# cloudflare/zkp-ecdsa

Measured on NVIDIA H100. Metric: ZKAttest proofs/sec, higher is better.
Workload: dtype u256/u258 (32-bit limbs, Montgomery)

## Files before the change

### zkp_ecdsa_b200/csrc/zk_curves.cuh

```cuda
#pragma once
#include "zk_field.cuh"

namespace zk {

#define WEI_PT P256Pt
#define WEI_AFF P256Aff
#define WEI_JAC P256Jac
#define WEI_F P256p
#define WEI_FN(n) p256_##n
#define WEI_B_MONT ZK_P256_B_MONT
#define WEI_GX_MONT ZK_P256_GX_MONT
#define WEI_GY_MONT ZK_P256_GY_MONT
#include "zk_weier.inc"
#undef WEI_PT
#undef WEI_AFF
#undef WEI_JAC
#undef WEI_F
#undef WEI_FN
#undef WEI_B_MONT
#undef WEI_GX_MONT
#undef WEI_GY_MONT

#if defined(ZKA_PG_WAR256)
#define WEI_PT WarPt
#define WEI_AFF WarAff
#define WEI_JAC WarJac
#define WEI_F Warp
#define WEI_FN(n) war_##n
#define WEI_B_MONT ZK_WAR_B_MONT
#define WEI_GX_MONT ZK_WAR_GX_MONT
#define WEI_GY_MONT ZK_WAR_GY_MONT
#include "zk_weier.inc"
#undef WEI_PT
#undef WEI_AFF
#undef WEI_JAC
#undef WEI_F
#undef WEI_FN
#undef WEI_B_MONT
#undef WEI_GX_MONT
#undef WEI_GY_MONT

enum : int { PGL = 8 };
using PGp = Warp;
using FpPG = FpWar;
using TomPt = WarPt;
using TomPre = WarAff;
using TompMsm = Warp;
using TompCommit = Warp;
ZK_HD void tom_set_identity(TomPt& p) { war_set_identity(p); }
ZK_HD void tom_from_affine(TomPt& p, const uint32_t* x, const uint32_t* y) {
  copy_n<8>(p.x, x);
  copy_n<8>(p.y, y);
  Warp::set_one(p.z);
}
ZK_HD void tom_set_generator(TomPt& p) {
  WarAff g;
  war_set_generator(g);
  war_from_affine(p, g);
}
ZK_HD bool tom_on_curve(const uint32_t* x, const uint32_t* y) { return war_on_curve(x, y); }
ZK_HD void tom_add(TomPt& r, const TomPt& p, const TomPt& q) { war_add(r, p, q); }
template <bool kNeedT, class F = Warp>
ZK_HD void tom_madd(TomPt& r, const TomPt& p, const TomPre& q) { war_madd(r, p, q); }
ZK_HD void tom_dbl(TomPt& r, const TomPt& p) { war_dbl(r, p); }
ZK_HD void tom_neg(TomPt& r, const TomPt& p) {
  copy_n<8>(r.x, p.x);
  Warp::neg(r.y, p.y);
  copy_n<8>(r.z, p.z);
}
ZK_HD void pg_dbl_n(TomPt& p, int c) { war_dbl_n(p, c); }
ZK_HD void pg_pre_neg(TomPre& q) { Warp::neg(q.y, q.y); }
ZK_HD bool pg_is_identity(const TomPt& p) { return war_is_identity(p); }
ZK_HD void pg_fixed_to_msm(TomPt&) {}
#else
struct TomPt {
  uint32_t x[9], y[9], t[9], z[9];
};
struct TomPre {
  uint32_t x[9], y[9], k[9];
};

ZK_HD void tom_const(uint32_t* r, int which) {
  constexpr uint32_t sa[9] = ZK_TOM_SQRTA_MONT;
  constexpr uint32_t isa[9] = ZK_TOM_INVSQRTA_MONT;
  constexpr uint32_t d1[9] = ZK_TOM_D1_MONT;
  constexpr uint32_t gx[9] = ZK_TOM_GX1_MONT;
  constexpr uint32_t gy[9] = ZK_TOM_GY_MONT;
  constexpr uint32_t s2[9] = ZK_TOM_SQRTND1_MONT;
  constexpr uint32_t is2[9] = ZK_TOM_INVSQRTND1_MONT;
  constexpr uint32_t dd2[9] = ZK_TOM_2D2_MONT;
  constexpr uint32_t isd[9] = ZK_TOM_INVSQRTND_MONT;
#pragma unroll
  for (int i = 0; i < 9; i++)
    r[i] = which == 0 ? sa[i] : which == 1 ? isa[i] : which == 2 ? d1[i] : which == 3 ? gx[i] : which == 4 ? gy[i]
           : which == 5 ? s2[i] : which == 6 ? is2[i] : which == 7 ? dd2[i] : isd[i];
}
enum { TOM_SQRTA = 0, TOM_INVSQRTA = 1, TOM_D1 = 2, TOM_GX1 = 3, TOM_GY = 4, TOM_SQRTND1 = 5, TOM_INVSQRTND1 = 6,
       TOM_2D2 = 7, TOM_INVSQRTND = 8 };

struct TompInl : Tomp {
  ZK_HD static void mul(uint32_t* r, const uint32_t* a, const uint32_t* b) {
#if defined(__CUDA_ARCH__) && !defined(ZKA_NO_PTX_MUL)
    ptx::tom_mul_body(r, a, b);
#else
    Tomp::mul(r, a, b);
#endif
  }
  ZK_HD static void sqr(uint32_t* r, const uint32_t* a) { mul(r, a, a); }
};
#if defined(ZKA_COMMIT_INLINE)
using TompCommit = TompInl;
#else
using TompCommit = Tomp;
#endif
#if defined(ZKA_MSM_INLINE)
using TompMsm = TompInl;
#else
using TompMsm = Tomp;
#endif

template <bool kNeedT, class F = Tomp>
ZK_HD void tom2_madd(TomPt& r, const TomPt& p, const TomPre& q) {
  uint32_t A[9], B[9], C[9], D[9], E[9], Fv[9], G[9], H[9];
  F::sub(A, p.y, p.x);
  F::mul(A, A, q.x);
  F::add(B, p.y, p.x);
  F::mul(B, B, q.y);
  F::mul(C, p.t, q.k);
  F::add(D, p.z, p.z);
  F::sub(E, B, A);
  F::sub(Fv, D, C);
  F::add(G, D, C);
  F::add(H, B, A);
  F::mul(r.x, E, Fv);
  F::mul(r.y, G, H);
  if (kNeedT) F::mul(r.t, E, H);
  F::mul(r.z, Fv, G);
}

ZK_HD void tom_set_identity(TomPt& p) {
  zero_n<9>(p.x);
  Tomp::set_one(p.y);
  zero_n<9>(p.t);
  Tomp::set_one(p.z);
}
ZK_HD void tom_from_affine(TomPt& p, const uint32_t* x1, const uint32_t* y) {
  copy_n<9>(p.x, x1);
  copy_n<9>(p.y, y);
  Tomp::mul(p.t, x1, y);
  Tomp::set_one(p.z);
}
ZK_HD void tom_set_generator(TomPt& p) {
  uint32_t gx[9], gy[9];
  tom_const(gx, TOM_GX1);
  tom_const(gy, TOM_GY);
  tom_from_affine(p, gx, gy);
}
ZK_HD bool tom_on_curve(const uint32_t* x1, const uint32_t* y) {
  using F = Tomp;
  uint32_t xx[9], yy[9], l[9], r[9], d1[9], one[9];
  F::sqr(xx, x1);
  F::sqr(yy, y);
  F::add(l, xx, yy);
  F::mul(r, xx, yy);
  tom_const(d1, TOM_D1);
  F::mul(r, r, d1);
  F::set_one(one);
  F::add(r, r, one);
  uint32_t d[9], o[9];
  F::sub(d, l, r);
  zero_n<9>(o);
  o[0] = 1;
  F::mul(d, d, o);
  uint32_t nz = 0, np = 0;
#pragma unroll
  for (int i = 0; i < 9; i++) { nz |= d[i]; np |= d[i] ^ FpTom::p(i); }
  return nz == 0 || np == 0;
}

ZK_HD void tom_add(TomPt& r, const TomPt& p, const TomPt& q) {
  using F = Tomp;
  uint32_t A[9], B[9], C[9], D[9], E[9], Fv[9], G[9], H[9], d1[9];
  tom_const(d1, TOM_D1);
  F::mul(A, p.x, q.x);
  F::mul(B, p.y, q.y);
  F::mul(C, p.t, q.t);
  F::mul(C, C, d1);
  F::mul(D, p.z, q.z);
  F::add(E, p.x, p.y);
  F::add(H, q.x, q.y);
  F::mul(E, E, H);
  F::sub(E, E, A);
  F::sub(E, E, B);
  F::sub(Fv, D, C);
  F::add(G, D, C);
  F::sub(H, B, A);
  F::mul(r.x, E, Fv);
  F::mul(r.y, G, H);
  F::mul(r.t, E, H);
  F::mul(r.z, Fv, G);
}
template <bool kNeedT, class F = Tomp>
ZK_HD void tom_madd(TomPt& r, const TomPt& p, const TomPre& q) {
  uint32_t A[9], B[9], C[9], E[9], Fv[9], G[9], H[9];
  F::mul(A, p.x, q.x);
  F::mul(B, p.y, q.y);
  F::mul(C, p.t, q.k);
  F::add(E, p.x, p.y);
  F::add(H, q.x, q.y);
  F::mul(E, E, H);
  F::sub(E, E, A);
  F::sub(E, E, B);
  F::sub(Fv, p.z, C);
  F::add(G, p.z, C);
  F::sub(H, B, A);
  F::mul(r.x, E, Fv);
  F::mul(r.y, G, H);
  if (kNeedT) F::mul(r.t, E, H);
  F::mul(r.z, Fv, G);
}
ZK_HD void tom_dbl(TomPt& r, const TomPt& p) {
  using F = Tomp;
  uint32_t A[9], B[9], C[9], E[9], G[9], Fv[9], H[9];
  F::sqr(A, p.x);
  F::sqr(B, p.y);
  F::sqr(C, p.z);
  F::add(C, C, C);
  F::add(E, p.x, p.y);
  F::sqr(E, E);
  F::sub(E, E, A);
  F::sub(E, E, B);
  F::add(G, A, B);
  F::sub(Fv, G, C);
  F::sub(H, A, B);
  F::mul(r.x, E, Fv);
  F::mul(r.y, G, H);
  F::mul(r.t, E, H);
  F::mul(r.z, Fv, G);
}
ZK_HD void tom_neg(TomPt& r, const TomPt& p) {
  Tomp::neg(r.x, p.x);
  copy_n<9>(r.y, p.y);
  Tomp::neg(r.t, p.t);
  copy_n<9>(r.z, p.z);
}


enum : int { PGL = 9 };
using PGp = Tomp;
using FpPG = FpTom;
ZK_HD void pg_dbl_n(TomPt& p, int c) {
  for (int i = 0; i < c; i++) tom_dbl(p, p);
}
ZK_HD void pg_pre_neg(TomPre& q) {
  Tomp::neg(q.x, q.x);
  Tomp::neg(q.k, q.k);
}
ZK_HD bool pg_is_identity(const TomPt& p) { return Tomp::is_zero(p.x) && Tomp::eq(p.y, p.z); }
ZK_HD void pg_fixed_to_msm(TomPt& f) {
  uint32_t cw[9], X[9], Y[9], Tt[9], Zp[9], c1[9];
  tom_const(c1, TOM_INVSQRTND1);
  Tomp::mul(cw, f.x, c1);
  Tomp::mul(X, cw, f.y);
  Tomp::sqr(Y, f.z);
  Tomp::mul(Tt, cw, f.z);
  Tomp::mul(Zp, f.z, f.y);
  copy_n<9>(f.x, X); copy_n<9>(f.y, Y); copy_n<9>(f.t, Tt); copy_n<9>(f.z, Zp);
}
#endif

}
```

### zkp_ecdsa_b200/csrc/zk_field_ptx.cuh

```cuda
#pragma once

#if defined(__CUDA_ARCH__)
namespace zk {
namespace ptx {

__device__ __forceinline__ void mac3(uint32_t& a0, uint32_t& a1, uint32_t& a2, uint32_t x, uint32_t y) {
  asm("mad.lo.cc.u32 %0, %3, %4, %0;\n\t"
      "madc.hi.cc.u32 %1, %3, %4, %1;\n\t"
      "addc.u32 %2, %2, 0;"
      : "+r"(a0), "+r"(a1), "+r"(a2)
      : "r"(x), "r"(y));
}
__device__ __forceinline__ void add3(uint32_t& a0, uint32_t& a1, uint32_t& a2, uint32_t lo, uint32_t hi) {
  asm("add.cc.u32 %0, %0, %3;\n\t"
      "addc.cc.u32 %1, %1, %4;\n\t"
      "addc.u32 %2, %2, 0;"
      : "+r"(a0), "+r"(a1), "+r"(a2)
      : "r"(lo), "r"(hi));
}
__device__ __forceinline__ void addw(uint32_t& a0, uint32_t& a1, uint32_t& a2, uint32_t w) {
  asm("add.cc.u32 %0, %0, %3;\n\t"
      "addc.cc.u32 %1, %1, 0;\n\t"
      "addc.u32 %2, %2, 0;"
      : "+r"(a0), "+r"(a1), "+r"(a2)
      : "r"(w));
}
__device__ __forceinline__ void subw(uint32_t& a0, uint32_t& a1, uint32_t& a2, uint32_t w) {
  asm("sub.cc.u32 %0, %0, %3;\n\t"
      "subc.cc.u32 %1, %1, 0;\n\t"
      "subc.u32 %2, %2, 0;"
      : "+r"(a0), "+r"(a1), "+r"(a2)
      : "r"(w));
}

__device__ __forceinline__ uint32_t shl_alu(uint32_t x, uint32_t n) {
  uint32_t r;
  asm("shf.l.clamp.b32 %0, %1, %2, %3;" : "=r"(r) : "r"(0u), "r"(x), "r"(n));
  return r;
}
__device__ __forceinline__ uint32_t shr_top_alu(uint32_t x, uint32_t n) {
  uint32_t r;
  asm("shf.l.clamp.b32 %0, %1, %2, %3;" : "=r"(r) : "r"(x), "r"(0u), "r"(n));
  return r;
}

__device__ __forceinline__ void tom_mul_body_ps(uint32_t* r, const uint32_t* a, const uint32_t* b) {
  constexpr int N = 9;
  constexpr uint32_t P0 = FpTom::p(0), P1 = FpTom::p(1), P2 = FpTom::p(2), P3 = FpTom::p(3), P7 = FpTom::p(7);
  static_assert(FpTom::p(4) == 2 && FpTom::p(5) == 0 && FpTom::p(6) == 4 && FpTom::p(8) == 3, "tom.p limb structure");
  uint32_t m[N], t[N];
  uint32_t a0 = 0, a1 = 0, a2 = 0;
#pragma unroll
  for (int k = 0; k < 2 * N; k++) {
#pragma unroll
    for (int i = 0; i < N; i++) {
      const int j = k - i;
      if (j >= 0 && j < N) mac3(a0, a1, a2, a[i], b[j]);
    }
#pragma unroll
    for (int i = 0; i < N; i++) {
      const int j = k - i;
      if (i < k && j >= 1 && j < N) {
        if (j == 1) mac3(a0, a1, a2, m[i], P1);
        else if (j == 2) mac3(a0, a1, a2, m[i], P2);
        else if (j == 3) mac3(a0, a1, a2, m[i], P3);
        else if (j == 7) mac3(a0, a1, a2, m[i], P7);
        else if (j == 4) add3(a0, a1, a2, shl_alu(m[i], 1), shr_top_alu(m[i], 1));
        else if (j == 6) add3(a0, a1, a2, shl_alu(m[i], 2), shr_top_alu(m[i], 2));
        else if (j == 8) { add3(a0, a1, a2, shl_alu(m[i], 1), shr_top_alu(m[i], 1)); add3(a0, a1, a2, m[i], 0u); }
      }
    }
    if (k < N) {
      m[k] = a0 * FpTom::kN0Inv;
      mac3(a0, a1, a2, m[k], P0);
    } else {
      t[k - N] = a0;
    }
    a0 = a1; a1 = a2; a2 = 0;
  }
#pragma unroll
  for (int i = 0; i < N; i++) r[i] = t[i];
}

template <int I, bool kFirst>
__device__ __forceinline__ void tom_row(uint32_t* A, uint32_t* Bq, uint32_t x, const uint32_t* b) {
  if (kFirst) {
    asm("mad.lo.cc.u32 %0, %9, %10, %0;\n\t"
        "madc.hi.cc.u32 %1, %9, %10, %1;\n\t"
        "madc.lo.cc.u32 %2, %9, %11, %2;\n\t"
        "madc.hi.cc.u32 %3, %9, %11, %3;\n\t"
        "madc.lo.cc.u32 %4, %9, %12, %4;\n\t"
        "madc.hi.cc.u32 %5, %9, %12, %5;\n\t"
        "madc.lo.cc.u32 %6, %9, %13, %6;\n\t"
        "madc.hi.cc.u32 %7, %9, %13, %7;\n\t"
        "addc.u32 %8, %8, 0;"
        : "+r"(Bq[I + 1]), "+r"(Bq[I + 2]), "+r"(Bq[I + 3]), "+r"(Bq[I + 4]), "+r"(Bq[I + 5]), "+r"(Bq[I + 6]),
          "+r"(Bq[I + 7]), "+r"(Bq[I + 8]), "+r"(Bq[I + 9])
        : "r"(x), "r"(b[1]), "r"(b[3]), "r"(b[5]), "r"(b[7]));
  } else {
    asm("add.cc.u32 %0, %0, %10;\n\t"
        "madc.lo.cc.u32 %1, %11, %12, %1;\n\t"
        "madc.hi.cc.u32 %2, %11, %12, %2;\n\t"
        "madc.lo.cc.u32 %3, %11, %13, %3;\n\t"
        "madc.hi.cc.u32 %4, %11, %13, %4;\n\t"
        "madc.lo.cc.u32 %5, %11, %14, %5;\n\t"
        "madc.hi.cc.u32 %6, %11, %14, %6;\n\t"
        "madc.lo.cc.u32 %7, %11, %15, %7;\n\t"
        "madc.hi.cc.u32 %8, %11, %15, %8;\n\t"
        "addc.u32 %9, %9, 0;"
        : "+r"(A[I]), "+r"(Bq[I + 1]), "+r"(Bq[I + 2]), "+r"(Bq[I + 3]), "+r"(Bq[I + 4]), "+r"(Bq[I + 5]),
          "+r"(Bq[I + 6]), "+r"(Bq[I + 7]), "+r"(Bq[I + 8]), "+r"(Bq[I + 9])
        : "r"(Bq[I]), "r"(x), "r"(b[1]), "r"(b[3]), "r"(b[5]), "r"(b[7]));
  }
  asm("mad.lo.cc.u32 %0, %11, %12, %0;\n\t"
      "madc.hi.cc.u32 %1, %11, %12, %1;\n\t"
      "madc.lo.cc.u32 %2, %11, %13, %2;\n\t"
      "madc.hi.cc.u32 %3, %11, %13, %3;\n\t"
      "madc.lo.cc.u32 %4, %11, %14, %4;\n\t"
      "madc.hi.cc.u32 %5, %11, %14, %5;\n\t"
      "madc.lo.cc.u32 %6, %11, %15, %6;\n\t"
      "madc.hi.cc.u32 %7, %11, %15, %7;\n\t"
      "madc.lo.cc.u32 %8, %11, %16, %8;\n\t"
      "madc.hi.u32 %9, %11, %16, %9;"
      : "+r"(A[I]), "+r"(A[I + 1]), "+r"(A[I + 2]), "+r"(A[I + 3]), "+r"(A[I + 4]), "+r"(A[I + 5]), "+r"(A[I + 6]),
        "+r"(A[I + 7]), "+r"(A[I + 8]), "+r"(A[I + 9]), "+r"(A[I + 10])
      : "r"(x), "r"(b[0]), "r"(b[2]), "r"(b[4]), "r"(b[6]), "r"(b[8]));
  const uint32_t m = A[I] * FpTom::kN0Inv;
  const uint32_t s1 = shl_alu(m, 1), t1 = shr_top_alu(m, 1), s2 = shl_alu(m, 2), t2 = shr_top_alu(m, 2);
  uint32_t lo3, hi3, lo7, hi7;
  asm("add.cc.u32 %0, %2, %3;\n\taddc.u32 %1, %4, 0;" : "=r"(lo3), "=r"(hi3) : "r"(s1), "r"(m), "r"(t1));
  asm("sub.cc.u32 %0, 0, %2;\n\tsubc.u32 %1, %3, %4;" : "=r"(lo7), "=r"(hi7) : "r"(s2), "r"(m), "r"(t2));
  constexpr uint32_t P0 = FpTom::p(0), P1 = FpTom::p(1), P2 = FpTom::p(2), P3 = FpTom::p(3);
  asm("mad.lo.cc.u32 %0, %11, %12, %0;\n\t"
      "madc.hi.cc.u32 %1, %11, %12, %1;\n\t"
      "madc.lo.cc.u32 %2, %11, %13, %2;\n\t"
      "madc.hi.cc.u32 %3, %11, %13, %3;\n\t"
      "addc.cc.u32 %4, %4, %14;\n\t"
      "addc.cc.u32 %5, %5, %15;\n\t"
      "addc.cc.u32 %6, %6, %16;\n\t"
      "addc.cc.u32 %7, %7, %17;\n\t"
      "addc.cc.u32 %8, %8, %18;\n\t"
      "addc.u32 %9, %9, %19;"
      : "+r"(A[I]), "+r"(A[I + 1]), "+r"(A[I + 2]), "+r"(A[I + 3]), "+r"(A[I + 4]), "+r"(A[I + 5]), "+r"(A[I + 6]),
        "+r"(A[I + 7]), "+r"(A[I + 8]), "+r"(A[I + 9]), "+r"(A[I + 10])
      : "r"(m), "r"(P0), "r"(P2), "r"(s1), "r"(t1), "r"(s2), "r"(t2), "r"(lo3), "r"(hi3));
  asm("mad.lo.cc.u32 %0, %9, %10, %0;\n\t"
      "madc.hi.cc.u32 %1, %9, %10, %1;\n\t"
      "madc.lo.cc.u32 %2, %9, %11, %2;\n\t"
      "madc.hi.cc.u32 %3, %9, %11, %3;\n\t"
      "addc.cc.u32 %4, %4, 0;\n\t"
      "addc.cc.u32 %5, %5, 0;\n\t"
      "addc.cc.u32 %6, %6, %12;\n\t"
      "addc.cc.u32 %7, %7, %13;\n\t"
      "addc.u32 %8, %8, 0;"
      : "+r"(Bq[I + 1]), "+r"(Bq[I + 2]), "+r"(Bq[I + 3]), "+r"(Bq[I + 4]), "+r"(Bq[I + 5]), "+r"(Bq[I + 6]),
        "+r"(Bq[I + 7]), "+r"(Bq[I + 8]), "+r"(Bq[I + 9])
      : "r"(m), "r"(P1), "r"(P3), "r"(lo7), "r"(hi7));
}
__device__ __forceinline__ void tom_mul_body(uint32_t* r, const uint32_t* a, const uint32_t* b) {
  static_assert(FpTom::p(4) == 2 && FpTom::p(5) == 0 && FpTom::p(6) == 4 && FpTom::p(7) == 0xfffffffcu && FpTom::p(8) == 3,
                "tom.p limb structure");
  uint32_t E[20], O[20];
#pragma unroll
  for (int i = 0; i < 20; i++) { E[i] = 0; O[i] = 0; }
  tom_row<0, true>(E, O, a[0], b);
  tom_row<1, false>(O, E, a[1], b);
  tom_row<2, false>(E, O, a[2], b);
  tom_row<3, false>(O, E, a[3], b);
  tom_row<4, false>(E, O, a[4], b);
  tom_row<5, false>(O, E, a[5], b);
  tom_row<6, false>(E, O, a[6], b);
  tom_row<7, false>(O, E, a[7], b);
  tom_row<8, false>(E, O, a[8], b);
  asm("add.cc.u32 %0, %9, %18;\n\t"
      "addc.cc.u32 %1, %10, %19;\n\t"
      "addc.cc.u32 %2, %11, %20;\n\t"
      "addc.cc.u32 %3, %12, %21;\n\t"
      "addc.cc.u32 %4, %13, %22;\n\t"
      "addc.cc.u32 %5, %14, %23;\n\t"
      "addc.cc.u32 %6, %15, %24;\n\t"
      "addc.cc.u32 %7, %16, %25;\n\t"
      "addc.u32 %8, %17, %26;"
      : "=r"(r[0]), "=r"(r[1]), "=r"(r[2]), "=r"(r[3]), "=r"(r[4]), "=r"(r[5]), "=r"(r[6]), "=r"(r[7]), "=r"(r[8])
      : "r"(E[9]), "r"(E[10]), "r"(E[11]), "r"(E[12]), "r"(E[13]), "r"(E[14]), "r"(E[15]), "r"(E[16]), "r"(E[17]),
        "r"(O[9]), "r"(O[10]), "r"(O[11]), "r"(O[12]), "r"(O[13]), "r"(O[14]), "r"(O[15]), "r"(O[16]), "r"(O[17]));
}

__device__ __forceinline__ void p256_mul_body(uint32_t* r, const uint32_t* a, const uint32_t* b) {
  constexpr int N = 8;
  uint32_t m[N], t[N + 1];
  uint32_t a0 = 0, a1 = 0, a2 = 0;
#pragma unroll
  for (int k = 0; k < 2 * N; k++) {
#pragma unroll
    for (int i = 0; i < N; i++) {
      const int j = k - i;
      if (j >= 0 && j < N) mac3(a0, a1, a2, a[i], b[j]);
    }
    if (k - 3 >= 0 && k - 3 < N) addw(a0, a1, a2, m[k - 3 < 0 ? 0 : (k - 3 >= N ? 0 : k - 3)]);
    if (k - 6 >= 0 && k - 6 < N) addw(a0, a1, a2, m[k - 6 < 0 ? 0 : (k - 6 >= N ? 0 : k - 6)]);
    if (k - 7 >= 0 && k - 7 < N) subw(a0, a1, a2, m[k - 7 < 0 ? 0 : (k - 7 >= N ? 0 : k - 7)]);
    if (k - 8 >= 0 && k - 8 < N) addw(a0, a1, a2, m[k - 8 < 0 ? 0 : (k - 8 >= N ? 0 : k - 8)]);
    if (k < N) {
      m[k] = a0;
      a0 = 0;
    } else {
      t[k - N] = a0;
    }
    a0 = a1; a1 = a2; a2 = (uint32_t)((int32_t)a2 >> 31);
  }
  t[N] = a0;
  uint32_t u[N];
  uint32_t br = sub_p<FpP256>(u, t);
  const bool ge = (t[N] != 0) || (br == 0);
#pragma unroll
  for (int i = 0; i < N; i++) r[i] = ge ? u[i] : t[i];
}

__device__ __forceinline__ void p256_sqr_body(uint32_t* r, const uint32_t* a) {
  constexpr int N = 8;
  uint32_t m[N], t[N + 1];
  uint32_t a0 = 0, a1 = 0, a2 = 0;
#pragma unroll
  for (int k = 0; k < 2 * N; k++) {
    if (k >= 1 && k <= 2 * N - 3) {
      uint32_t c0 = 0, c1 = 0, c2 = 0;
#pragma unroll
      for (int i = 0; i < N; i++) {
        const int j = k - i;
        if (i < j && j < N) mac3(c0, c1, c2, a[i], a[j]);
      }
      asm("add.cc.u32 %0, %0, %0;\n\t"
          "addc.cc.u32 %1, %1, %1;\n\t"
          "addc.u32 %2, %2, %2;\n\t"
          "add.cc.u32 %3, %3, %0;\n\t"
          "addc.cc.u32 %4, %4, %1;\n\t"
          "addc.u32 %5, %5, %2;"
          : "+r"(c0), "+r"(c1), "+r"(c2), "+r"(a0), "+r"(a1), "+r"(a2));
    }
    if ((k & 1) == 0 && k / 2 < N) mac3(a0, a1, a2, a[k / 2], a[k / 2]);
    if (k - 3 >= 0 && k - 3 < N) addw(a0, a1, a2, m[k - 3 < 0 ? 0 : (k - 3 >= N ? 0 : k - 3)]);
    if (k - 6 >= 0 && k - 6 < N) addw(a0, a1, a2, m[k - 6 < 0 ? 0 : (k - 6 >= N ? 0 : k - 6)]);
    if (k - 7 >= 0 && k - 7 < N) subw(a0, a1, a2, m[k - 7 < 0 ? 0 : (k - 7 >= N ? 0 : k - 7)]);
    if (k - 8 >= 0 && k - 8 < N) addw(a0, a1, a2, m[k - 8 < 0 ? 0 : (k - 8 >= N ? 0 : k - 8)]);
    if (k < N) {
      m[k] = a0;
      a0 = 0;
    } else {
      t[k - N] = a0;
    }
    a0 = a1; a1 = a2; a2 = (uint32_t)((int32_t)a2 >> 31);
  }
  t[N] = a0;
  uint32_t u[N];
  uint32_t br = sub_p<FpP256>(u, t);
  const bool ge = (t[N] != 0) || (br == 0);
#pragma unroll
  for (int i = 0; i < N; i++) r[i] = ge ? u[i] : t[i];
}

template <int I, bool kFirst>
__device__ __forceinline__ void p256_row(uint32_t* A, uint32_t* Bq, uint32_t x, const uint32_t* b) {
  if (kFirst) {
    asm("mad.lo.cc.u32 %0, %9, %10, %0;\n\t"
        "madc.hi.cc.u32 %1, %9, %10, %1;\n\t"
        "madc.lo.cc.u32 %2, %9, %11, %2;\n\t"
        "madc.hi.cc.u32 %3, %9, %11, %3;\n\t"
        "madc.lo.cc.u32 %4, %9, %12, %4;\n\t"
        "madc.hi.cc.u32 %5, %9, %12, %5;\n\t"
        "madc.lo.cc.u32 %6, %9, %13, %6;\n\t"
        "madc.hi.cc.u32 %7, %9, %13, %7;\n\t"
        "addc.u32 %8, %8, 0;"
        : "+r"(Bq[I + 1]), "+r"(Bq[I + 2]), "+r"(Bq[I + 3]), "+r"(Bq[I + 4]), "+r"(Bq[I + 5]), "+r"(Bq[I + 6]),
          "+r"(Bq[I + 7]), "+r"(Bq[I + 8]), "+r"(Bq[I + 9])
        : "r"(x), "r"(b[1]), "r"(b[3]), "r"(b[5]), "r"(b[7]));
  } else {
    asm("add.cc.u32 %0, %0, %10;\n\t"
        "madc.lo.cc.u32 %1, %11, %12, %1;\n\t"
        "madc.hi.cc.u32 %2, %11, %12, %2;\n\t"
        "madc.lo.cc.u32 %3, %11, %13, %3;\n\t"
        "madc.hi.cc.u32 %4, %11, %13, %4;\n\t"
        "madc.lo.cc.u32 %5, %11, %14, %5;\n\t"
        "madc.hi.cc.u32 %6, %11, %14, %6;\n\t"
        "madc.lo.cc.u32 %7, %11, %15, %7;\n\t"
        "madc.hi.cc.u32 %8, %11, %15, %8;\n\t"
        "addc.u32 %9, %9, 0;"
        : "+r"(A[I]), "+r"(Bq[I + 1]), "+r"(Bq[I + 2]), "+r"(Bq[I + 3]), "+r"(Bq[I + 4]), "+r"(Bq[I + 5]),
          "+r"(Bq[I + 6]), "+r"(Bq[I + 7]), "+r"(Bq[I + 8]), "+r"(Bq[I + 9])
        : "r"(Bq[I]), "r"(x), "r"(b[1]), "r"(b[3]), "r"(b[5]), "r"(b[7]));
  }
  asm("mad.lo.cc.u32 %0, %9, %10, %0;\n\t"
      "madc.hi.cc.u32 %1, %9, %10, %1;\n\t"
      "madc.lo.cc.u32 %2, %9, %11, %2;\n\t"
      "madc.hi.cc.u32 %3, %9, %11, %3;\n\t"
      "madc.lo.cc.u32 %4, %9, %12, %4;\n\t"
      "madc.hi.cc.u32 %5, %9, %12, %5;\n\t"
      "madc.lo.cc.u32 %6, %9, %13, %6;\n\t"
      "madc.hi.cc.u32 %7, %9, %13, %7;\n\t"
      "addc.u32 %8, %8, 0;"
      : "+r"(A[I]), "+r"(A[I + 1]), "+r"(A[I + 2]), "+r"(A[I + 3]), "+r"(A[I + 4]), "+r"(A[I + 5]), "+r"(A[I + 6]),
        "+r"(A[I + 7]), "+r"(A[I + 8])
      : "r"(x), "r"(b[0]), "r"(b[2]), "r"(b[4]), "r"(b[6]));
  const uint32_t m = A[I];
  uint32_t negm, third;
  asm("sub.cc.u32 %0, 0, %2;\n\tsubc.u32 %1, %2, 0;" : "=r"(negm), "=r"(third) : "r"(m));
  asm("add.cc.u32 %0, %0, %7;\n\t"
      "addc.cc.u32 %1, %1, 0;\n\t"
      "addc.cc.u32 %2, %2, 0;\n\t"
      "addc.cc.u32 %3, %3, %7;\n\t"
      "addc.cc.u32 %4, %4, %8;\n\t"
      "addc.cc.u32 %5, %5, %9;\n\t"
      "addc.u32 %6, %6, 0;"
      : "+r"(A[I + 3]), "+r"(A[I + 4]), "+r"(A[I + 5]), "+r"(A[I + 6]), "+r"(A[I + 7]), "+r"(A[I + 8]), "+r"(A[I + 9])
      : "r"(m), "r"(negm), "r"(third));
}
__device__ __forceinline__ void p256_mul_body_os(uint32_t* r, const uint32_t* a, const uint32_t* b) {
  constexpr int N = 8;
  uint32_t E[18], O[18];
#pragma unroll
  for (int i = 0; i < 18; i++) { E[i] = 0; O[i] = 0; }
  p256_row<0, true>(E, O, a[0], b);
  p256_row<1, false>(O, E, a[1], b);
  p256_row<2, false>(E, O, a[2], b);
  p256_row<3, false>(O, E, a[3], b);
  p256_row<4, false>(E, O, a[4], b);
  p256_row<5, false>(O, E, a[5], b);
  p256_row<6, false>(E, O, a[6], b);
  p256_row<7, false>(O, E, a[7], b);
  uint32_t t[N + 1];
  asm("add.cc.u32 %0, %9, %18;\n\t"
      "addc.cc.u32 %1, %10, %19;\n\t"
      "addc.cc.u32 %2, %11, %20;\n\t"
      "addc.cc.u32 %3, %12, %21;\n\t"
      "addc.cc.u32 %4, %13, %22;\n\t"
      "addc.cc.u32 %5, %14, %23;\n\t"
      "addc.cc.u32 %6, %15, %24;\n\t"
      "addc.cc.u32 %7, %16, %25;\n\t"
      "addc.u32 %8, %17, %26;"
// ... 68 lines not shown
```

### zkp_ecdsa_b200/csrc/zk_ops.cuh

```cuda
#pragma once
#include "zk_curves.cuh"
#include "zk_layout.h"
#include "zk_sha256.cuh"

namespace zk {

#if defined(__CUDA_ARCH__)
#define ZK_SET_STATUS(ptr, code) atomicCAS((int*)(ptr), 0, (int)(code))
#define ZK_SET_STATUS_OVER(ptr, code, over) \
  do {                                      \
    atomicCAS((int*)(ptr), 0, (int)(code)); \
    atomicCAS((int*)(ptr), (int)(over), (int)(code)); \
  } while (0)
#else
#define ZK_SET_STATUS_OVER(ptr, code, over)              \
  do {                                                   \
    if (*(ptr) == 0 || *(ptr) == (over)) *(ptr) = (code); \
  } while (0)
#define ZK_SET_STATUS(ptr, code) \
  do {                           \
    if (*(ptr) == 0) *(ptr) = (code); \
  } while (0)
#endif

// ... 342 lines not shown
      tom_add(acc, acc, p);
    }
  }
};
struct TomTabE2Task {
  const uint32_t* proj;
  uint32_t* pre;
  int count;
  ZK_HD void operator()(int t) const {
    using F = Tomp;
    constexpr int CH = 16;
    const int lo = t * CH;
    int n = count - lo;
    if (n > CH) n = CH;
    if (n <= 0) return;
    uint32_t pf[CH][9];
    uint32_t acc[9], y[9], z[9], den[9];
    F::set_one(acc);
    for (int k = 0; k < n; k++) {
      const uint32_t* src = proj + (size_t)(lo + k) * TOM_PROJ_WORDS;
      uint32_t xx[9];
      tom_ld_xyz(xx, y, z, src);
      F::mul(den, y, z);
      F::mul(acc, acc, den);
      copy_n<9>(pf[k], acc);
    }
    uint32_t inv[9], s2[9], dd2[9];
    F::inv(inv, acc);
    tom_const(s2, TOM_SQRTND1);
    tom_const(dd2, TOM_2D2);
    for (int k = n - 1; k >= 0; k--) {
      const uint32_t* src = proj + (size_t)(lo + k) * TOM_PROJ_WORDS;
      uint32_t x[9], di[9], w[9], v[9], kk[9], ym[9], yp[9];
      tom_ld_xyz(x, y, z, src);
      F::mul(den, y, z);
      if (k > 0) F::mul(di, inv, pf[k - 1]); else copy_n<9>(di, inv);
      F::mul(inv, inv, den);
      F::mul(w, x, y);
      F::mul(w, w, di);
      F::mul(w, w, s2);
      F::sqr(v, z);
      F::mul(v, v, di);
      F::mul(kk, w, v);
      F::mul(kk, kk, dd2);
      F::sub(ym, v, w);
      F::add(yp, v, w);
      F::reduce(ym); F::reduce(yp); F::reduce(kk);
      uint32_t* o = pre + (size_t)(lo + k) * TOM_PRE_WORDS;
      st<9>(o, ym); st<9>(o + 9, yp); st<9>(o + 18, kk);
      for (int i = 27; i < 32; i++) o[i] = 0;
    }
  }
};

struct TomNormTask {
  const uint32_t* proj;
  uint32_t* aff;
  uint8_t* bytes;
  int count;
  int chunk;
  int e2;
  int aff_mod, aff_lim;
  ZK_HD static void canon2p(uint32_t* r) {
    uint32_t t[9], p2[9];
#pragma unroll
    for (int i = 0; i < 9; i++) p2[i] = (FpTom::p(i) << 1) | (i > 0 ? (FpTom::p(i - 1) >> 31) : 0u);
    uint32_t br = sub_n<9>(t, r, p2);
    csel_n<9>(r, br == 0, t, r);
    br = sub_p<FpTom>(t, r);
    csel_n<9>(r, br == 0, t, r);
  }
  ZK_HD void operator()(int t) const {
    using F = Tomp;
    const int lo = t * chunk;
    int n = count - lo;
    if (n > chunk) n = chunk;
    if (n <= 0) return;
    uint32_t pre[NORM_CHUNK_MAX][9];
    uint32_t acc[9], z[9], v[9], den[9];
    F::set_one(acc);
    for (int k = 0; k < n; k++) {
      const uint32_t* src = proj + (size_t)(lo + k) * TOM_PROJ_WORDS;
      uint32_t xx[9];
      tom_ld_xyz(xx, v, z, src);
      if (e2) F::mul(den, z, v); else copy_n<9>(den, z);
      F::mul(acc, acc, den);
      copy_n<9>(pre[k], acc);
    }
    uint32_t inv[9], isa[9], is2[9], isd[9], one_plain[9];
    F::inv(inv, acc);
    tom_const(isa, TOM_INVSQRTA);
    tom_const(is2, TOM_INVSQRTND1);
    tom_const(isd, TOM_INVSQRTND);
    zero_n<9>(one_plain);
    one_plain[0] = 1;
    for (int k = n - 1; k >= 0; k--) {
      const uint32_t* src = proj + (size_t)(lo + k) * TOM_PROJ_WORDS;
      uint32_t X[9], Y[9], di[9];
      tom_ld_xyz(X, Y, z, src);
      if (e2) F::mul(den, z, Y); else copy_n<9>(den, z);
      if (k > 0) F::mul(di, inv, pre[k - 1]); else copy_n<9>(di, inv);
      F::mul(inv, inv, den);
      if (bytes) {
        uint32_t Dp[9], cx[9], cy[9];
        F::mul(Dp, di, one_plain);
        if (e2) {
          F::mul(cx, X, Y);
          F::mul(cx, cx, isd);
          F::mul(cx, cx, Dp);
          F::sqr(cy, z);
          F::mul(cy, cy, Dp);
        } else {
          F::mul(cx, X, isa);
          F::mul(cx, cx, Dp);
          F::mul(cy, Y, Dp);
        }
        canon2p(cx);
        canon2p(cy);
        store_point_words<9, 33>(bytes + (size_t)(lo + k) * BSTRIDE, 0x04u, cx, cy);
      }
      if (aff && ((lo + k) % aff_mod) < aff_lim) {
        uint32_t x[9], y[9];
        if (e2) {
          uint32_t zi[9], vi[9];
          F::mul(zi, di, Y);
          F::mul(vi, di, z);
          F::mul(x, X, zi);
          F::mul(x, x, is2);
          F::mul(y, z, vi);
        } else {
          F::mul(x, X, di);
          F::mul(y, Y, di);
        }
        uint32_t* a = aff + (size_t)(lo + k) * TOM_AFF_WORDS;
        st<9>(a, x);
        st<9>(a + 9, y);
      }
    }
  }
};

struct TomCommitTask {
  const uint32_t* jv;
  const uint32_t* jr;
  const uint32_t* gtab;
  const uint32_t* htab;
  uint32_t* proj;
  int w, nwin;
  ZK_HD void operator()(int t) const {
    uint32_t v[8], r[8];
    ld<8>(v, jv + (size_t)t * 8);
    ld<8>(r, jr + (size_t)t * 8);
    TomPt acc;
    tom_set_identity(acc);
    const size_t ne = (size_t)fb_entries(w);
    uint32_t cv = 0, cr = 0;
    for (int j = 0; j < nwin; j++) {
      TomPre q;
      bool nv, nr;
      const uint32_t dv = signed_digit(v, j, w, cv, nv), dr = signed_digit(r, j, w, cr, nr);
      tom_ld_pre(q, gtab + ((size_t)j * ne + dv) * TOM_PRE_WORDS);
      tom2_pre_neg(q, nv);
      tom2_madd<true>(acc, acc, q);
      tom_ld_pre(q, htab + ((size_t)j * ne + dr) * TOM_PRE_WORDS);
      tom2_pre_neg(q, nr);
      tom2_madd<true>(acc, acc, q);
    }
    uint32_t* o = proj + (size_t)t * TOM_PROJ_WORDS;
    tom_st_xyz(o, acc.x, acc.y, acc.z);
  }
};

struct TomCommitGTask {
  const uint32_t* jv;
  const uint32_t* gtab;
  uint32_t* ext;
  int w, nwin;
  ZK_HD void operator()(int t) const {
    const int item = t / GJOBS_PER_ITEM, g = t % GJOBS_PER_ITEM;
    uint32_t v[8];
    ld<8>(v, jv + ((size_t)item * JOBS_PER_ITEM + item_job_of_gpart(g)) * 8);
    TomPt acc;
    tom_set_identity(acc);
    const size_t ne = (size_t)fb_entries(w);
    uint32_t carry = 0;
#pragma unroll 1
    for (int j = 0; j < nwin; j++) {
      TomPre q;
      bool neg;
      const uint32_t d = signed_digit(v, j, w, carry, neg);
      tom_ld_pre(q, gtab + ((size_t)j * ne + d) * TOM_PRE_WORDS);
      tom2_pre_neg(q, neg);
      tom2_madd<true, TompCommit>(acc, acc, q);
    }
    uint32_t* o = ext + (size_t)t * TOM_EXT_WORDS;
    st<9>(o, acc.x); st<9>(o + 9, acc.y); st<9>(o + 18, acc.t); st<9>(o + 27, acc.z);
  }
};
struct TomCommitHTask {
  const uint32_t* jr;
  const uint32_t* htab;
  const uint32_t* ext;
  uint32_t* proj;
  int w, nwin;
  ZK_HD void operator()(int t) const {
    const int item = t / JOBS_PER_ITEM, jb = t % JOBS_PER_ITEM;
    uint32_t r[8];
    ld<8>(r, jr + (size_t)t * 8);
    TomPt acc;
    const uint32_t* s = ext + ((size_t)item * GJOBS_PER_ITEM + item_gpart_of_job(jb)) * TOM_EXT_WORDS;
    ld<9>(acc.x, s); ld<9>(acc.y, s + 9); ld<9>(acc.t, s + 18); ld<9>(acc.z, s + 27);
    const size_t ne = (size_t)fb_entries(w);
    uint32_t carry = 0;
#pragma unroll 1
    for (int j = 0; j < nwin; j++) {
      TomPre q;
      bool neg;
      const uint32_t d = signed_digit(r, j, w, carry, neg);
      tom_ld_pre(q, htab + ((size_t)j * ne + d) * TOM_PRE_WORDS);
      tom2_pre_neg(q, neg);
      tom2_madd<true, TompCommit>(acc, acc, q);
    }
    tom_st_xyz(proj + (size_t)t * TOM_PROJ_WORDS, acc.x, acc.y, acc.z);
  }
};

#if !defined(ZKA_HOSTSIM) && defined(ZKA_COMMIT_MINBLOCKS)
template <> struct TaskMinBlocks<TomCommitHTask> { static constexpr int value = ZKA_COMMIT_MINBLOCKS; };
template <> struct TaskMinBlocks<TomCommitGTask> { static constexpr int value = ZKA_COMMIT_MINBLOCKS; };
template <> struct TaskMinBlocks<TomCommitTask> { static constexpr int value = ZKA_COMMIT_MINBLOCKS; };
#endif

#endif

enum : int { GK_BLOCK_BITS = 10 };
ZK_HD int gk_block_bits(int n) { return n < GK_BLOCK_BITS ? n : GK_BLOCK_BITS; }
ZK_HD void gk_block_sum(uint32_t* acc, const uint32_t* ring_m, const uint32_t (*fz)[8], const uint32_t (*fo)[8], int n,
                        int k, uint32_t blk, const uint32_t* vw) {
  using F = Tomq;
  uint32_t P[21][8];
  F::set_one(P[n]);
  for (int j = n - 1; j >= k; j--) F::mul(P[j], P[j + 1], ((blk >> (j - k)) & 1u) ? fo[j] : fz[j]);
  for (int j = k - 1; j >= 0; j--) F::mul(P[j], P[j + 1], fz[j]);
  zero_n<8>(acc);
  const size_t base = (size_t)blk << k;
  const uint32_t cnt = 1u << k;
  for (uint32_t l = 0;;) {
    uint32_t vi[8], term[8];
    ld<8>(vi, ring_m + (base + l) * 8);
    if (vw) F::sub(vi, vw, vi);
    F::mul(term, vi, P[0]);
    F::add(acc, acc, term);
    l++;
    if (l == cnt) break;
    int tz = 0;
    while (!((l >> tz) & 1u)) tz++;
    F::mul(P[tz], P[tz + 1], fo[tz]);
    for (int j = tz - 1; j >= 0; j--) F::mul(P[j], P[j + 1], fz[j]);
  }
}

ZK_HD bool hash_pt_fetch(uint32_t* t, const uint8_t* p, int len) {
  if (((size_t)p & 3) || len < 64 || len > 68) return false;
  if (aligned16(p)) {
#pragma unroll
    for (int j = 0; j < 4; j++) ld4(t + 4 * j, p + 16 * j);
    t[16] = len > 64 ? *reinterpret_cast<const uint32_t*>(p + 64) : 0u;
    return true;
  }
  const uint32_t* q = reinterpret_cast<const uint32_t*>(p);
#pragma unroll
  for (int j = 0; j < 17; j++) t[j] = (4 * j < len) ? q[j] : 0u;
  return true;
}
template <class Src>
ZK_HD void hash_points80(uint32_t* c3, const Src& src, int npts) {
  Sha256 h;
  h.init();
  uint32_t nx[17], cu[17];
  int nlen = 0;
  const uint8_t* np = npts > 0 ? src(0, nlen) : nullptr;
  bool nfast = npts > 0 && hash_pt_fetch(nx, np, nlen);
  for (int i = 0; i < npts; i++) {
    const uint8_t* p = np;
    const int len = nlen;
    const bool fast = nfast;
#pragma unroll
    for (int j = 0; j < 17; j++) cu[j] = nx[j];
    if (i + 1 < npts) {
      np = src(i + 1, nlen);
      nfast = hash_pt_fetch(nx, np, nlen);
    }
    if (fast) h.feed17(cu, len);
    else h.update(p, len);
  }
  h.final80(c3);
}

ZK_HD void challenge_to_limbs(uint32_t* r, const uint32_t* c3) {
  zero_n<8>(r);
  r[0] = c3[0]; r[1] = c3[1]; r[2] = c3[2];
}

template <int N>
ZK_HD void load_point(uint32_t* w, const uint8_t* src) {
  if (aligned16(src)) {
#pragma unroll
    for (int j = 0; j < BSTRIDE / 16; j++) ld4(w + 4 * j, src + 16 * j);
  } else if (((size_t)src & 3) == 0) {
    const uint32_t* sw = reinterpret_cast<const uint32_t*>(src);
#pragma unroll
    for (int j = 0; j < BSTRIDE / 4; j++) w[j] = 4 * j < N ? sw[j] : 0u;
  } else {
#pragma unroll
    for (int j = 0; j < BSTRIDE / 4; j++) {
      uint32_t v = 0;
#pragma unroll
      for (int t = 0; t < 4; t++)
        if (4 * j + t < N) v |= (uint32_t)src[4 * j + t] << (8 * t);
      w[j] = v;
    }
  }
}

struct ByteWriter {
  uint8_t* blk;
  uint32_t q[4];
  int fill;
  int lead;
  ZK_HD explicit ByteWriter(uint8_t* dst) : blk(dst - ((size_t)dst & 15)), fill((int)((size_t)dst & 15)), lead(fill) {
    q[0] = q[1] = q[2] = q[3] = 0;
  }
  ZK_HD static uint32_t funnel(uint32_t lo, uint32_t hi, int sh) {
#if defined(__CUDA_ARCH__)
    return __funnelshift_l(lo, hi, sh);
#else
    return (uint32_t)((((uint64_t)hi << 32) | lo) >> (32 - sh));
#endif
  }
  ZK_HD void store_part(int lo, int hi) const {
#pragma unroll
    for (int w = 0; w < 4; w++) {
      if (lo <= 4 * w && 4 * w + 4 <= hi) {
        *reinterpret_cast<uint32_t*>(blk + 4 * w) = q[w];
      } else {
#pragma unroll
        for (int t = 0; t < 4; t++)
          if (lo <= 4 * w + t && 4 * w + t < hi) blk[4 * w + t] = (uint8_t)(q[w] >> (8 * t));
      }
    }
  }
  ZK_HD void chunk(const uint32_t* c, int nb) {
    uint32_t m[4];
#pragma unroll
    for (int i = 0; i < 4; i++) {
      const int k = nb - 4 * i;
      m[i] = k >= 4 ? c[i] : k <= 0 ? 0u : c[i] & ((1u << (8 * k)) - 1u);
    }
    const int sh = 8 * (fill & 3), ws = fill >> 2;
    uint32_t d[5];
    d[0] = sh ? m[0] << sh : m[0];
#pragma unroll
    for (int i = 1; i < 4; i++) d[i] = funnel(m[i - 1], m[i], sh);
    d[4] = sh ? m[3] >> (32 - sh) : 0u;
    uint32_t e[8];
#pragma unroll
    for (int k = 0; k < 8; k++) {
      uint32_t v = 0;
#pragma unroll
      for (int s = 0; s < 4; s++)
        if (k - s >= 0 && k - s <= 4) v = ws == s ? d[k - s] : v;
      e[k] = v;
    }
#pragma unroll
// ... 54 lines not shown
```

Measured before the change: 92360.

## Defer Montgomery sparse-prime correction and skip identity madd and final T in commits

Restructures the Tom-field PTX Montgomery multiply. Each row now folds fewer terms of the sparse modulus and defers part of the reduction into a single shifted subtraction over the collected m values at the end; the first row uses plain multiplies instead of accumulating into zeroed arrays. The commit kernels also replace the first mixed add from the identity with a cheaper start routine, and skip computing T on the last madd. This removes per-row ALU work and some wasted field multiplications, at the risk of subtle carry or bound errors in the deferred reduction.

```diff
diff --git a/zkp_ecdsa_b200/csrc/zk_curves.cuh b/zkp_ecdsa_b200/csrc/zk_curves.cuh
--- a/zkp_ecdsa_b200/csrc/zk_curves.cuh
+++ b/zkp_ecdsa_b200/csrc/zk_curves.cuh
@@ -120,7 +120,7 @@
 #endif
 
 template <bool kNeedT, class F = Tomp>
-ZK_HD void tom2_madd(TomPt& r, const TomPt& p, const TomPre& q) {
+ZK_HD void tom2_madd(TomPt& r, const TomPt& p, const TomPre& q, bool need_t = true) {
   uint32_t A[9], B[9], C[9], D[9], E[9], Fv[9], G[9], H[9];
   F::sub(A, p.y, p.x);
   F::mul(A, A, q.x);
@@ -134,8 +134,23 @@
   F::add(H, B, A);
   F::mul(r.x, E, Fv);
   F::mul(r.y, G, H);
-  if (kNeedT) F::mul(r.t, E, H);
-  F::mul(r.z, Fv, G);
+  if (kNeedT && need_t) F::mul(r.t, E, H);
+  F::mul(r.z, Fv, G);
+}
+ZK_HD void tom2_start(TomPt& r, const TomPre& q) {
+  using F = Tomp;
+  uint32_t pp[9], t[9], d[9], s[9], one[9];
+#pragma unroll
+  for (int i = 0; i < 9; i++) pp[i] = FpTom::p(i);
+  add_n<9>(t, q.y, pp);
+  sub_n<9>(d, t, q.x);
+  F::add(s, q.y, q.x);
+  F::add(r.x, d, d);
+  F::add(r.y, s, s);
+  F::mul(r.t, d, s);
+  F::set_one(one);
+  F::add(r.z, one, one);
+  F::add(r.z, r.z, r.z);
 }
 
 ZK_HD void tom_set_identity(TomPt& p) {
diff --git a/zkp_ecdsa_b200/csrc/zk_field_ptx.cuh b/zkp_ecdsa_b200/csrc/zk_field_ptx.cuh
--- a/zkp_ecdsa_b200/csrc/zk_field_ptx.cuh
+++ b/zkp_ecdsa_b200/csrc/zk_field_ptx.cuh
@@ -82,22 +82,34 @@
   for (int i = 0; i < N; i++) r[i] = t[i];
 }
 
-template <int I, bool kFirst>
-__device__ __forceinline__ void tom_row(uint32_t* A, uint32_t* Bq, uint32_t x, const uint32_t* b) {
-  if (kFirst) {
-    asm("mad.lo.cc.u32 %0, %9, %10, %0;\n\t"
-        "madc.hi.cc.u32 %1, %9, %10, %1;\n\t"
-        "madc.lo.cc.u32 %2, %9, %11, %2;\n\t"
-        "madc.hi.cc.u32 %3, %9, %11, %3;\n\t"
-        "madc.lo.cc.u32 %4, %9, %12, %4;\n\t"
-        "madc.hi.cc.u32 %5, %9, %12, %5;\n\t"
-        "madc.lo.cc.u32 %6, %9, %13, %6;\n\t"
-        "madc.hi.cc.u32 %7, %9, %13, %7;\n\t"
-        "addc.u32 %8, %8, 0;"
-        : "+r"(Bq[I + 1]), "+r"(Bq[I + 2]), "+r"(Bq[I + 3]), "+r"(Bq[I + 4]), "+r"(Bq[I + 5]), "+r"(Bq[I + 6]),
-          "+r"(Bq[I + 7]), "+r"(Bq[I + 8]), "+r"(Bq[I + 9])
+template <int I>
+__device__ __forceinline__ void tom_row(uint32_t* A, uint32_t* Bq, uint32_t x, const uint32_t* b, uint32_t& m) {
+  if constexpr (I == 0) {
+    asm("mul.lo.u32 %0, %8, %9;\n\t"
+        "mul.hi.u32 %1, %8, %9;\n\t"
+        "mul.lo.u32 %2, %8, %10;\n\t"
+        "mul.hi.u32 %3, %8, %10;\n\t"
+        "mul.lo.u32 %4, %8, %11;\n\t"
+        "mul.hi.u32 %5, %8, %11;\n\t"
+        "mul.lo.u32 %6, %8, %12;\n\t"
+        "mul.hi.u32 %7, %8, %12;"
+        : "=r"(Bq[1]), "=r"(Bq[2]), "=r"(Bq[3]), "=r"(Bq[4]), "=r"(Bq[5]), "=r"(Bq[6]), "=r"(Bq[7]), "=r"(Bq[8])
         : "r"(x), "r"(b[1]), "r"(b[3]), "r"(b[5]), "r"(b[7]));
+    asm("mul.lo.u32 %0, %10, %11;\n\t"
+        "mul.hi.u32 %1, %10, %11;\n\t"
+        "mul.lo.u32 %2, %10, %12;\n\t"
+        "mul.hi.u32 %3, %10, %12;\n\t"
+        "mul.lo.u32 %4, %10, %13;\n\t"
+        "mul.hi.u32 %5, %10, %13;\n\t"
+        "mul.lo.u32 %6, %10, %14;\n\t"
+        "mul.hi.u32 %7, %10, %14;\n\t"
+        "mul.lo.u32 %8, %10, %15;\n\t"
+        "mul.hi.u32 %9, %10, %15;"
+        : "=r"(A[0]), "=r"(A[1]), "=r"(A[2]), "=r"(A[3]), "=r"(A[4]), "=r"(A[5]), "=r"(A[6]), "=r"(A[7]),
+          "=r"(A[8]), "=r"(A[9])
+        : "r"(x), "r"(b[0]), "r"(b[2]), "r"(b[4]), "r"(b[6]), "r"(b[8]));
   } else {
+    uint32_t c1;
     asm("add.cc.u32 %0, %0, %10;\n\t"
         "madc.lo.cc.u32 %1, %11, %12, %1;\n\t"
         "madc.hi.cc.u32 %2, %11, %12, %2;\n\t"
@@ -107,71 +119,78 @@
         "madc.hi.cc.u32 %6, %11, %14, %6;\n\t"
         "madc.lo.cc.u32 %7, %11, %15, %7;\n\t"
         "madc.hi.cc.u32 %8, %11, %15, %8;\n\t"
-        "addc.u32 %9, %9, 0;"
+        "addc.u32 %9, 0, 0;"
         : "+r"(A[I]), "+r"(Bq[I + 1]), "+r"(Bq[I + 2]), "+r"(Bq[I + 3]), "+r"(Bq[I + 4]), "+r"(Bq[I + 5]),
-          "+r"(Bq[I + 6]), "+r"(Bq[I + 7]), "+r"(Bq[I + 8]), "+r"(Bq[I + 9])
+          "+r"(Bq[I + 6]), "+r"(Bq[I + 7]), "+r"(Bq[I + 8]), "=r"(c1)
         : "r"(Bq[I]), "r"(x), "r"(b[1]), "r"(b[3]), "r"(b[5]), "r"(b[7]));
-  }
-  asm("mad.lo.cc.u32 %0, %11, %12, %0;\n\t"
-      "madc.hi.cc.u32 %1, %11, %12, %1;\n\t"
-      "madc.lo.cc.u32 %2, %11, %13, %2;\n\t"
-      "madc.hi.cc.u32 %3, %11, %13, %3;\n\t"
-      "madc.lo.cc.u32 %4, %11, %14, %4;\n\t"
-      "madc.hi.cc.u32 %5, %11, %14, %5;\n\t"
-      "madc.lo.cc.u32 %6, %11, %15, %6;\n\t"
-      "madc.hi.cc.u32 %7, %11, %15, %7;\n\t"
-      "madc.lo.cc.u32 %8, %11, %16, %8;\n\t"
-      "madc.hi.u32 %9, %11, %16, %9;"
+    asm("mad.lo.cc.u32 %0, %10, %11, %0;\n\t"
+        "madc.hi.cc.u32 %1, %10, %11, %1;\n\t"
+        "madc.lo.cc.u32 %2, %10, %12, %2;\n\t"
+        "madc.hi.cc.u32 %3, %10, %12, %3;\n\t"
+        "madc.lo.cc.u32 %4, %10, %13, %4;\n\t"
+        "madc.hi.cc.u32 %5, %10, %13, %5;\n\t"
+        "madc.lo.cc.u32 %6, %10, %14, %6;\n\t"
+        "madc.hi.cc.u32 %7, %10, %14, %7;\n\t"
+        "madc.lo.cc.u32 %8, %10, %15, %8;\n\t"
+        "madc.hi.u32 %9, %10, %15, %16;"
+        : "+r"(A[I]), "+r"(A[I + 1]), "+r"(A[I + 2]), "+r"(A[I + 3]), "+r"(A[I + 4]), "+r"(A[I + 5]), "+r"(A[I + 6]),
+          "+r"(A[I + 7]), "+r"(A[I + 8]), "=r"(A[I + 9])
+        : "r"(x), "r"(b[0]), "r"(b[2]), "r"(b[4]), "r"(b[6]), "r"(b[8]), "r"(c1));
+  }
+  m = A[I] * FpTom::kN0Inv;
+  const uint32_t s1 = shl_alu(m, 1), t1 = shr_top_alu(m, 1), s2 = shl_alu(m, 2), t2 = shr_top_alu(m, 2);
+  constexpr uint32_t P0 = FpTom::p(0), P1 = FpTom::p(1), P2 = FpTom::p(2), P3 = FpTom::p(3);
+  asm("mad.lo.cc.u32 %0, %10, %11, %0;\n\t"
+      "madc.hi.cc.u32 %1, %10, %11, %1;\n\t"
+      "madc.lo.cc.u32 %2, %10, %12, %2;\n\t"
+      "madc.hi.cc.u32 %3, %10, %12, %3;\n\t"
+      "addc.cc.u32 %4, %4, %13;\n\t"
+      "addc.cc.u32 %5, %5, %14;\n\t"
+      "addc.cc.u32 %6, %6, %15;\n\t"
+      "addc.cc.u32 %7, %7, %16;\n\t"
+      "addc.cc.u32 %8, %8, %15;\n\t"
+      "addc.u32 %9, %9, %16;"
       : "+r"(A[I]), "+r"(A[I + 1]), "+r"(A[I + 2]), "+r"(A[I + 3]), "+r"(A[I + 4]), "+r"(A[I + 5]), "+r"(A[I + 6]),
-        "+r"(A[I + 7]), "+r"(A[I + 8]), "+r"(A[I + 9]), "+r"(A[I + 10])
-      : "r"(x), "r"(b[0]), "r"(b[2]), "r"(b[4]), "r"(b[6]), "r"(b[8]));
-  const uint32_t m = A[I] * FpTom::kN0Inv;
-  const uint32_t s1 = shl_alu(m, 1), t1 = shr_top_alu(m, 1), s2 = shl_alu(m, 2), t2 = shr_top_alu(m, 2);
-  uint32_t lo3, hi3, lo7, hi7;
-  asm("add.cc.u32 %0, %2, %3;\n\taddc.u32 %1, %4, 0;" : "=r"(lo3), "=r"(hi3) : "r"(s1), "r"(m), "r"(t1));
-  asm("sub.cc.u32 %0, 0, %2;\n\tsubc.u32 %1, %3, %4;" : "=r"(lo7), "=r"(hi7) : "r"(s2), "r"(m), "r"(t2));
-  constexpr uint32_t P0 = FpTom::p(0), P1 = FpTom::p(1), P2 = FpTom::p(2), P3 = FpTom::p(3);
-  asm("mad.lo.cc.u32 %0, %11, %12, %0;\n\t"
-      "madc.hi.cc.u32 %1, %11, %12, %1;\n\t"
-      "madc.lo.cc.u32 %2, %11, %13, %2;\n\t"
-      "madc.hi.cc.u32 %3, %11, %13, %3;\n\t"
-      "addc.cc.u32 %4, %4, %14;\n\t"
-      "addc.cc.u32 %5, %5, %15;\n\t"
-      "addc.cc.u32 %6, %6, %16;\n\t"
-      "addc.cc.u32 %7, %7, %17;\n\t"
-      "addc.cc.u32 %8, %8, %18;\n\t"
-      "addc.u32 %9, %9, %19;"
-      : "+r"(A[I]), "+r"(A[I + 1]), "+r"(A[I + 2]), "+r"(A[I + 3]), "+r"(A[I + 4]), "+r"(A[I + 5]), "+r"(A[I + 6]),
-        "+r"(A[I + 7]), "+r"(A[I + 8]), "+r"(A[I + 9]), "+r"(A[I + 10])
-      : "r"(m), "r"(P0), "r"(P2), "r"(s1), "r"(t1), "r"(s2), "r"(t2), "r"(lo3), "r"(hi3));
+        "+r"(A[I + 7]), "+r"(A[I + 8]), "+r"(A[I + 9])
+      : "r"(m), "r"(P0), "r"(P2), "r"(s1), "r"(t1), "r"(s2), "r"(t2));
+  if constexpr (I < 2) {
+    asm("sub.cc.u32 %0, %0, %3;\n\t"
+        "subc.cc.u32 %1, %1, %4;\n\t"
+        "subc.u32 %2, %2, 0;"
+        : "+r"(A[I + 7]), "+r"(A[I + 8]), "+r"(A[I + 9])
+        : "r"(s2), "r"(t2));
+  }
   asm("mad.lo.cc.u32 %0, %9, %10, %0;\n\t"
       "madc.hi.cc.u32 %1, %9, %10, %1;\n\t"
       "madc.lo.cc.u32 %2, %9, %11, %2;\n\t"
       "madc.hi.cc.u32 %3, %9, %11, %3;\n\t"
       "addc.cc.u32 %4, %4, 0;\n\t"
       "addc.cc.u32 %5, %5, 0;\n\t"
-      "addc.cc.u32 %6, %6, %12;\n\t"
-      "addc.cc.u32 %7, %7, %13;\n\t"
-      "addc.u32 %8, %8, 0;"
+      "addc.cc.u32 %6, %6, 0;\n\t"
+      "addc.cc.u32 %7, %7, 0;\n\t"
+      "addc.u32 %8, 0, 0;"
       : "+r"(Bq[I + 1]), "+r"(Bq[I + 2]), "+r"(Bq[I + 3]), "+r"(Bq[I + 4]), "+r"(Bq[I + 5]), "+r"(Bq[I + 6]),
-        "+r"(Bq[I + 7]), "+r"(Bq[I + 8]), "+r"(Bq[I + 9])
-      : "r"(m), "r"(P1), "r"(P3), "r"(lo7), "r"(hi7));
+        "+r"(Bq[I + 7]), "+r"(Bq[I + 8]), "=r"(Bq[I + 9])
+      : "r"(m), "r"(P1), "r"(P3));
 }
 __device__ __forceinline__ void tom_mul_body(uint32_t* r, const uint32_t* a, const uint32_t* b) {
   static_assert(FpTom::p(4) == 2 && FpTom::p(5) == 0 && FpTom::p(6) == 4 && FpTom::p(7) == 0xfffffffcu && FpTom::p(8) == 3,
                 "tom.p limb structure");
-  uint32_t E[20], O[20];
-#pragma unroll
-  for (int i = 0; i < 20; i++) { E[i] = 0; O[i] = 0; }
-  tom_row<0, true>(E, O, a[0], b);
-  tom_row<1, false>(O, E, a[1], b);
-  tom_row<2, false>(E, O, a[2], b);
-  tom_row<3, false>(O, E, a[3], b);
-  tom_row<4, false>(E, O, a[4], b);
-  tom_row<5, false>(O, E, a[5], b);
-  tom_row<6, false>(E, O, a[6], b);
-  tom_row<7, false>(O, E, a[7], b);
-  tom_row<8, false>(E, O, a[8], b);
+  uint32_t E[18], O[18], m[9];
+  tom_row<0>(E, O, a[0], b, m[0]);
+  tom_row<1>(O, E, a[1], b, m[1]);
+  tom_row<2>(E, O, a[2], b, m[2]);
+  tom_row<3>(O, E, a[3], b, m[3]);
+  tom_row<4>(E, O, a[4], b, m[4]);
+  tom_row<5>(O, E, a[5], b, m[5]);
+  tom_row<6>(E, O, a[6], b, m[6]);
+  tom_row<7>(O, E, a[7], b, m[7]);
+  tom_row<8>(E, O, a[8], b, m[8]);
+  uint32_t s[8];
+  s[0] = shl_alu(m[2], 2);
+#pragma unroll
+  for (int k = 1; k < 7; k++) asm("shf.l.wrap.b32 %0, %1, %2, 2;" : "=r"(s[k]) : "r"(m[k + 1]), "r"(m[k + 2]));
+  s[7] = shr_top_alu(m[8], 2);
   asm("add.cc.u32 %0, %9, %18;\n\t"
       "addc.cc.u32 %1, %10, %19;\n\t"
       "addc.cc.u32 %2, %11, %20;\n\t"
@@ -184,6 +203,17 @@
       : "=r"(r[0]), "=r"(r[1]), "=r"(r[2]), "=r"(r[3]), "=r"(r[4]), "=r"(r[5]), "=r"(r[6]), "=r"(r[7]), "=r"(r[8])
       : "r"(E[9]), "r"(E[10]), "r"(E[11]), "r"(E[12]), "r"(E[13]), "r"(E[14]), "r"(E[15]), "r"(E[16]), "r"(E[17]),
         "r"(O[9]), "r"(O[10]), "r"(O[11]), "r"(O[12]), "r"(O[13]), "r"(O[14]), "r"(O[15]), "r"(O[16]), "r"(O[17]));
+  asm("sub.cc.u32 %0, %0, %9;\n\t"
+      "subc.cc.u32 %1, %1, %10;\n\t"
+      "subc.cc.u32 %2, %2, %11;\n\t"
+      "subc.cc.u32 %3, %3, %12;\n\t"
+      "subc.cc.u32 %4, %4, %13;\n\t"
+      "subc.cc.u32 %5, %5, %14;\n\t"
+      "subc.cc.u32 %6, %6, %15;\n\t"
+      "subc.cc.u32 %7, %7, %16;\n\t"
+      "subc.u32 %8, %8, 0;"
+      : "+r"(r[0]), "+r"(r[1]), "+r"(r[2]), "+r"(r[3]), "+r"(r[4]), "+r"(r[5]), "+r"(r[6]), "+r"(r[7]), "+r"(r[8])
+      : "r"(s[0]), "r"(s[1]), "r"(s[2]), "r"(s[3]), "r"(s[4]), "r"(s[5]), "r"(s[6]), "r"(s[7]));
 }
 
 __device__ __forceinline__ void p256_mul_body(uint32_t* r, const uint32_t* a, const uint32_t* b) {
diff --git a/zkp_ecdsa_b200/csrc/zk_ops.cuh b/zkp_ecdsa_b200/csrc/zk_ops.cuh
--- a/zkp_ecdsa_b200/csrc/zk_ops.cuh
+++ b/zkp_ecdsa_b200/csrc/zk_ops.cuh
@@ -518,7 +518,6 @@
     ld<8>(v, jv + (size_t)t * 8);
     ld<8>(r, jr + (size_t)t * 8);
     TomPt acc;
-    tom_set_identity(acc);
     const size_t ne = (size_t)fb_entries(w);
     uint32_t cv = 0, cr = 0;
     for (int j = 0; j < nwin; j++) {
@@ -527,10 +526,11 @@
       const uint32_t dv = signed_digit(v, j, w, cv, nv), dr = signed_digit(r, j, w, cr, nr);
       tom_ld_pre(q, gtab + ((size_t)j * ne + dv) * TOM_PRE_WORDS);
       tom2_pre_neg(q, nv);
-      tom2_madd<true>(acc, acc, q);
+      if (j == 0) tom2_start(acc, q);
+      else tom2_madd<true>(acc, acc, q);
       tom_ld_pre(q, htab + ((size_t)j * ne + dr) * TOM_PRE_WORDS);
       tom2_pre_neg(q, nr);
-      tom2_madd<true>(acc, acc, q);
+      tom2_madd<true>(acc, acc, q, j + 1 < nwin);
     }
     uint32_t* o = proj + (size_t)t * TOM_PROJ_WORDS;
     tom_st_xyz(o, acc.x, acc.y, acc.z);
@@ -547,7 +547,6 @@
     uint32_t v[8];
     ld<8>(v, jv + ((size_t)item * JOBS_PER_ITEM + item_job_of_gpart(g)) * 8);
     TomPt acc;
-    tom_set_identity(acc);
     const size_t ne = (size_t)fb_entries(w);
     uint32_t carry = 0;
 #pragma unroll 1
@@ -557,7 +556,8 @@
       const uint32_t d = signed_digit(v, j, w, carry, neg);
       tom_ld_pre(q, gtab + ((size_t)j * ne + d) * TOM_PRE_WORDS);
       tom2_pre_neg(q, neg);
-      tom2_madd<true, TompCommit>(acc, acc, q);
+      if (j == 0) tom2_start(acc, q);
+      else tom2_madd<true, TompCommit>(acc, acc, q);
     }
     uint32_t* o = ext + (size_t)t * TOM_EXT_WORDS;
     st<9>(o, acc.x); st<9>(o + 9, acc.y); st<9>(o + 18, acc.t); st<9>(o + 27, acc.z);
@@ -585,7 +585,7 @@
       const uint32_t d = signed_digit(r, j, w, carry, neg);
       tom_ld_pre(q, htab + ((size_t)j * ne + d) * TOM_PRE_WORDS);
       tom2_pre_neg(q, neg);
-      tom2_madd<true, TompCommit>(acc, acc, q);
+      tom2_madd<true, TompCommit>(acc, acc, q, j + 1 < nwin);
     }
     tom_st_xyz(proj + (size_t)t * TOM_PROJ_WORDS, acc.x, acc.y, acc.z);
   }
```

After: 96340 (median of 6 runs). 4.3% higher.
